# MachinePerceptionLab/Attentive_DFPrior

Hardware: AMD Instinct MI355X
Metric: rendered rays/sec (64 samples/ray), Replica room0 (higher is better)
Workload: dtype f32 via f16x3 split (3 f16 MFMA products per f32 product: 22-bit products, f32 accumulate); 1 GPU; room0 640x480 render_img, 64 spp (48+16), synthetic box room, seed-0 random decoders, grids at the REFERENCE init (N(0,.01), high N(0,1e-4)); stage color, ray_batch_size 100000 (per-batch far clamp, rendered as one call with a depth maximum per 100 000-ray segment), ONE frame per step; samples_per_ray=64

## Files before the change

### attentive_dfprior_amd/csrc/adfp_decode_g.h

```cpp
#pragma once
#include "adfp_decode_h.h"

__host__ __device__ constexpr int unit16(int k) { return 16 * ((k & 7) >> 2) + 4 * (k >> 3) + (k & 3); }

template <int CDIM, int NOUT>
struct DecLayoutG {
    using F = DecLayout<CDIM, NOUT>;
    static constexpr int KG_E = 3;
    static constexpr int KG_C = CDIM / 32;
    __host__ __device__ static constexpr int kg(int i) { return i == 0 ? KG_E : (i == 3 ? KG_E + 1 : 1); }
    static constexpr int P_BM = 0;
    __host__ __device__ static constexpr int layer_words(int i) { return kg(i) * 1024 + 32 + KG_C * 1024 + 32; }
    __host__ __device__ static constexpr int P_WP(int i) {
        int o = 384;
        for (int k = 0; k < i; ++k) o += layer_words(k);
        return o;
    }
    __host__ __device__ static constexpr int P_BP(int i) { return P_WP(i) + kg(i) * 1024; }
    __host__ __device__ static constexpr int P_WC(int i) { return P_BP(i) + 32; }
    __host__ __device__ static constexpr int P_BC(int i) { return P_WC(i) + KG_C * 1024; }
    static constexpr int P_WO = P_WP(5);
    static constexpr int P_BO = P_WO + NOUT * 32;
    static constexpr int P_FLAG = P_BO + 4;
    static constexpr int NFLAG = (((P_FLAG + 511) / 256) + 3) & ~3;
    static constexpr int P_TOTAL = P_FLAG + NFLAG;
    static_assert((P_TOTAL + 255) / 256 <= NFLAG, "one flag word per pack block");
};

template <int CDIM, int NOUT>
__device__ HSrc dec_g_src(int t) {
    using L = DecLayoutG<CDIM, NOUT>;
    using F = DecLayout<CDIM, NOUT>;
    if (t < 384) {
        const int row = t >> 2, c = t & 3;
        const int f = (row & ~31) + unit16(row & 31);
        return HSrc{0, (f < 93 && c < 3) ? F::F_EB + c * 93 + f : -1, -1};
    }
#pragma unroll
    for (int i = 0; i < 5; ++i) {
        if (t < L::P_BP(i) || (t >= L::P_WC(i) && t < L::P_BC(i))) {
            const bool fc = t >= L::P_WC(i);
            const int u = t - (fc ? L::P_WC(i) : L::P_WP(i));
            const int grp = u >> 10, ob = (u >> 9) & 1, part = (u >> 8) & 1, g = (u >> 6) & 3, row = 16 * ob + ((u >> 2) & 15), jp = (u & 3) * 2;
            int src[2];
#pragma unroll
            for (int e = 0; e < 2; ++e) {
                int col = 32 * grp + unit16(8 * g + jp + e);
                if (fc) src[e] = F::F_FC(i) + row * CDIM + col;
                else {
                    if (i == 0) { if (col >= 93) col = -1; }
                    else if (i == 3) { if (col < 96) { if (col >= 93) col = -1; } else col = 93 + (col - 96); }
                    src[e] = col < 0 ? -1 : F::F_PL(i) + row * F::in_dim(i) + col;
                }
            }
            return HSrc{1 + part, src[0], src[1]};
        }
        if (t < L::P_WC(i)) return HSrc{0, F::F_PL(i) + 32 * F::in_dim(i) + (t - L::P_BP(i)), -1};
        if (t < L::P_BC(i) + 32) return HSrc{0, F::F_FC(i) + 32 * CDIM + (t - L::P_BC(i)), -1};
    }
    if (t < L::P_BO) {
        const int u = t - L::P_WO;
        return HSrc{0, F::F_OW + u, -1};
    }
    const int o = t - L::P_BO;
    return HSrc{0, o < NOUT ? F::F_OB + o : -1, -1};
}

template <int CDIM, int NOUT>
ADFP_DEV void pack_decoder_g_block(int blk, const float* __restrict__ flat, unsigned* __restrict__ packed, int* __restrict__ status, int bit) {
    using L = DecLayoutG<CDIM, NOUT>;
    const int t = blk * 256 + (int)threadIdx.x;
    HSrc s{0, -1, -1};
    float a = 0.f, b = 0.f;
    if (t < L::P_FLAG) {
        s = dec_g_src<CDIM, NOUT>(t);
        a = s.s0 < 0 ? 0.f : flat[s.s0]; b = s.s1 < 0 ? 0.f : flat[s.s1];
    }
    pack_block_flag(!(fmaxf(fabsf(a), fabsf(b)) < 65504.0f), packed + L::P_FLAG + blk, status, bit);
    if (t >= L::P_FLAG) return;
    if (s.kind == 0) { packed[t] = s.s0 < 0 ? 0u : __float_as_uint(a); return; }
    a = f16_clamp(a); b = f16_clamp(b);
    const float ah = f16_hi_part(a), bh = f16_hi_part(b);
    _Float16 x, y;
    if (s.kind == 1) { x = (_Float16)ah; y = (_Float16)bh; }
    else { x = (_Float16)(a - ah); y = (_Float16)(b - bh); }
    packed[t] = (unsigned)__builtin_bit_cast(unsigned short, x) | ((unsigned)__builtin_bit_cast(unsigned short, y) << 16);
}
template <int CDIM, int NOUT>
__global__ void k_pack_decoder_g(const float* __restrict__ flat, unsigned* __restrict__ packed, int* __restrict__ status, int bit) { pack_decoder_g_block<CDIM, NOUT>((int)blockIdx.x, flat, packed, status, bit); }

typedef float f32x4g __attribute__((ext_vector_type(4)));

ADFP_DEV void swap_halves(float& x, float& y) {
    const auto r = __builtin_amdgcn_permlane32_swap(__float_as_uint(x), __float_as_uint(y), false, false);
    x = __uint_as_float(r[0]); y = __uint_as_float(r[1]);
}

template <int NG>
ADFP_DEV void mfma_chain_g(f32x4g acc[2][2], const unsigned* __restrict__ w, const f16x8 (*xh)[2], const f16x8 (*xl)[2]) {
#pragma unroll
    for (int kg = 0; kg < NG; ++kg) {
#pragma unroll
        for (int ob = 0; ob < 2; ++ob) {
            const f16x8 ah = __builtin_bit_cast(f16x8, *(const u32x4*)(w + kg * 1024 + ob * 512));
            const f16x8 al = __builtin_bit_cast(f16x8, *(const u32x4*)(w + kg * 1024 + ob * 512 + 256));
#pragma unroll
            for (int pb = 0; pb < 2; ++pb) {
                acc[ob][pb] = __builtin_amdgcn_mfma_f32_16x16x32_f16(ah, xh[kg][pb], acc[ob][pb], 0, 0, 0);
                acc[ob][pb] = __builtin_amdgcn_mfma_f32_16x16x32_f16(ah, xl[kg][pb], acc[ob][pb], 0, 0, 0);
                acc[ob][pb] = __builtin_amdgcn_mfma_f32_16x16x32_f16(al, xh[kg][pb], acc[ob][pb], 0, 0, 0);
            }
        }
    }
    __builtin_amdgcn_sched_barrier(0);
}

ADFP_DEV void row_store(float* p, const f32x4 v) {
    *(f32x4*)p = v;
}
template <int CDIM, int NOUT, int TRAIN = 0>
ADFP_DEV void decode_net_g(const unsigned* __restrict__ ldsu, const GridDev& grid, const GridDev& grid1, const float pn[3], const float (*pf)[3],
                           int lane, float& amax, float (*out)[NOUT], unsigned* __restrict__ mw, float* srow0, unsigned rowbits) {
    using L = DecLayoutG<CDIM, NOUT>;
    using ST = DecStage<CDIM>;
    const int g = lane >> 4;
    float* srow[2] = {nullptr, nullptr};
    if constexpr (TRAIN) {
        srow[0] = (rowbits & 1u) ? srow0 : nullptr;
        srow[1] = (rowbits & 2u) ? srow0 + 16 * ST::NXM : nullptr;
    }
    const unsigned* wl = ldsu + 4 * lane;
    const float* b4 = (const float*)ldsu + 4 * g;
    const float* brow = (const float*)ldsu + 32 * g;
    f16x8 ch[L::KG_C][2], cl[L::KG_C][2];
#pragma unroll
    for (int kc = 0; kc < L::KG_C; ++kc) {
        float c[16];
        gather16(kc == 0 ? grid : grid1, pn, g & 1, c);
        float x[8] = {c[0], c[1], c[2], c[3], c[8], c[9], c[10], c[11]};
        float y[8] = {c[4], c[5], c[6], c[7], c[12], c[13], c[14], c[15]};
#pragma unroll
        for (int s = 0; s < 8; ++s) swap_halves(x[s], y[s]);
        if constexpr (TRAIN) {
            static_assert(!TRAIN || CDIM == 32, "training rows: 32-channel decoders");
            if (srow[0]) { row_store(srow[0] + ST::xm(ST::SC) + 4 * g, f32x4{x[0], x[1], x[2], x[3]}); row_store(srow[0] + ST::xm(ST::SC) + 16 + 4 * g, f32x4{x[4], x[5], x[6], x[7]}); }
            if (srow[1]) { row_store(srow[1] + ST::xm(ST::SC) + 4 * g, f32x4{y[0], y[1], y[2], y[3]}); row_store(srow[1] + ST::xm(ST::SC) + 16 + 4 * g, f32x4{y[4], y[5], y[6], y[7]}); }
        }
        split8(x, ch[kc][0], cl[kc][0], amax);
        split8(y, ch[kc][1], cl[kc][1], amax);
    }
    f16x8 eh[L::KG_E][2], el[L::KG_E][2];
#pragma unroll
    for (int kg = 0; kg < L::KG_E; ++kg) {
        float e0[8], e1[8];
#pragma unroll
        for (int j = 0; j < 8; ++j) {
            const f32x4 bm = *(const f32x4*)(brow + L::P_BM + (32 * kg + j) * 4);
            e0[j] = adfp_sinf(fmaf(pf[0][2], bm.z, fmaf(pf[0][1], bm.y, pf[0][0] * bm.x)));
            e1[j] = adfp_sinf(fmaf(pf[1][2], bm.z, fmaf(pf[1][1], bm.y, pf[1][0] * bm.x)));
        }
        split8<false>(e0, eh[kg][0], el[kg][0], amax);
        split8<false>(e1, eh[kg][1], el[kg][1], amax);
    }
    __builtin_amdgcn_sched_barrier(0);
    f32x4g acc[2][2];
    f16x8 hh[1][2], hl[1][2];
    unsigned mk[3] = {0u, 0u, 0u};
#pragma unroll
    for (int i = 0; i < 5; ++i) {
#pragma unroll
        for (int ob = 0; ob < 2; ++ob) { const f32x4 t = *(const f32x4*)(b4 + L::P_BP(i) + 16 * ob); acc[ob][0] = t; acc[ob][1] = t; }
        if (i == 0) mfma_chain_g<L::KG_E>(acc, wl + L::P_WP(0), eh, el);
        else if (i == 3) {
            mfma_chain_g<L::KG_E>(acc, wl + L::P_WP(3), eh, el);
            mfma_chain_g<1>(acc, wl + L::P_WP(3) + L::KG_E * 1024, hh, hl);
        } else mfma_chain_g<1>(acc, wl + L::P_WP(i), hh, hl);
#pragma unroll
        for (int ob = 0; ob < 2; ++ob) {
            const f32x4 t = *(const f32x4*)(b4 + L::P_BC(i) + 16 * ob);
#pragma unroll
            for (int pb = 0; pb < 2; ++pb)
#pragma unroll
                for (int r = 0; r < 4; ++r) {
                    const float v = relu_f(acc[ob][pb][r]);
                    if constexpr (TRAIN) mk[i >> 1] = __builtin_amdgcn_alignbit(mk[i >> 1], 0u - __float_as_uint(v), 31);
                    acc[ob][pb][r] = v + t[r];
                }
        }
        mfma_chain_g<L::KG_C>(acc, wl + L::P_WC(i), ch, cl);
        if constexpr (TRAIN) {
#pragma unroll
            for (int pb = 0; pb < 2; ++pb) if (srow[pb]) {
                row_store(srow[pb] + ST::xm(ST::SH(i)) + 4 * g, f32x4{acc[0][pb][0], acc[0][pb][1], acc[0][pb][2], acc[0][pb][3]});
                row_store(srow[pb] + ST::xm(ST::SH(i)) + 16 + 4 * g, f32x4{acc[1][pb][0], acc[1][pb][1], acc[1][pb][2], acc[1][pb][3]});
            }
        }
        if (i < 4) {
#pragma unroll
            for (int pb = 0; pb < 2; ++pb) {
                const float t[8] = {acc[0][pb][0], acc[0][pb][1], acc[0][pb][2], acc[0][pb][3],
                                    acc[1][pb][0], acc[1][pb][1], acc[1][pb][2], acc[1][pb][3]};
                split8(t, hh[0][pb], hl[0][pb], amax);
            }
        }
    }
#pragma unroll
    for (int o = 0; o < NOUT; ++o) {
        const f32x4 w0 = *(const f32x4*)(b4 + L::P_WO + 32 * o), w1 = *(const f32x4*)(b4 + L::P_WO + 32 * o + 16);
#pragma unroll
        for (int pb = 0; pb < 2; ++pb) {
            float s = 0.f;
#pragma unroll
            for (int r = 0; r < 4; ++r) s = fmaf(acc[0][pb][r], w0[r], s);
#pragma unroll
            for (int r = 0; r < 4; ++r) s = fmaf(acc[1][pb][r], w1[r], s);
            s += __shfl_xor(s, 16);
            s += __shfl_xor(s, 32);
            out[pb][o] = s + ((const float*)ldsu)[L::P_BO + o];
        }
    }
    if constexpr (TRAIN) {
        const int sh = 4 * (g >> 1);
        unsigned wpb[2][3];
#pragma unroll
        for (int pb = 0; pb < 2; ++pb) {
            unsigned f[5];
#pragma unroll
            for (int i = 0; i < 5; ++i) {
                const unsigned m16 = (i == 4 || (i & 1)) ? (mk[i >> 1] & 0xFFFFu) : (mk[i >> 1] >> 16);
                const unsigned n0 = (m16 >> (12 - 4 * pb)) & 0xFu, n1 = (m16 >> (4 - 4 * pb)) & 0xFu;
                f[i] = (n0 << (12 - sh)) | (n1 << (4 - sh));
            }
            wpb[pb][0] = f[0] | (f[1] << 16); wpb[pb][1] = f[2] | (f[3] << 16); wpb[pb][2] = f[4];
        }
#pragma unroll
        for (int k = 0; k < 3; ++k) {
            const auto r = __builtin_amdgcn_permlane32_swap(wpb[0][k], wpb[1][k], false, false);
            mw[k] = r[0] | r[1];
        }
    }
}

template <int NT>
__global__ __launch_bounds__(NT, NT / 256) void k_decode_lc16(DecodeLCArgs a) {
    using LL = DecLayoutG<32, 1>;
    using LC = DecLayoutG<32, 4>;
    __shared__ __attribute__((aligned(16))) unsigned lds_all[LL::P_TOTAL + LC::P_TOTAL];
    __shared__ int s_next;
    __shared__ unsigned long long s_ring[ADFP_POOL_RING];
    unsigned* lds_low = lds_all;
    unsigned* lds_col = lds_all + LL::P_TOTAL;
    image_to_lds<NT, LL::P_TOTAL / 4>(lds_low, a.packed_low);
    image_to_lds<NT, LC::P_TOTAL / 4>(lds_col, a.packed_color);
    if (threadIdx.x == 0) s_next = NT / 64;
    if (threadIdx.x < ADFP_POOL_RING) s_ring[threadIdx.x] = 0ull;
    __syncthreads();
    const int lane = threadIdx.x & 63, n = lane & 15, g = lane >> 4;
    const int count = a.P.n;
    const int ntiles = (count + 31) >> 5;
    const TilePlan plan = tile_plan(ntiles, (int)gridDim.x, NT / 64, a.pool != nullptr);
    float amax_low = image_out_of_range<LL::P_FLAG, LL::NFLAG>(lds_low) ? INFINITY : 0.f;
    float amax_col = image_out_of_range<LC::P_FLAG, LC::NFLAG>(lds_col) ? INFINITY : 0.f;
    for (int j = threadIdx.x >> 6, tile; (tile = claim_tile_pool<NT / 64>(j, &s_next, s_ring, plan, ntiles, a.pool, a.status)) >= 0;) {
        const int idx = tile * 32 + 16 * (g >> 1) + n;
        const bool valid = idx < count;
        const int q = valid ? idx : 0;
        float pn[3], pf[2][3];
        bool pnan, keep_occ;
        {
            double pt[3];
            load_point(a.P, q, pt);
            normalize3(a.nb, pt, pn);
            const float f0 = (float)pt[0], f1 = (float)pt[1], f2 = (float)pt[2];
            pnan = (pt[0] != pt[0]) | (pt[1] != pt[1]) | (pt[2] != pt[2]);
            const unsigned f = a.flags ? a.flags[q] : 0u;
            keep_occ = (f & ADFP_F_BAND) || in_bound(pt, a.b) || !a.apply_bound;
            pf[0][0] = f0; pf[0][1] = f1; pf[0][2] = f2; pf[1][0] = f0; pf[1][1] = f1; pf[1][2] = f2;
        }
#pragma unroll
        for (int k = 0; k < 3; ++k) swap_halves(pf[0][k], pf[1][k]);
        float occ[2][1], rgb[2][4];
        int off_low = 0, off_col = LL::P_TOTAL;
        asm volatile("" : "+v"(off_low), "+v"(off_col));
        decode_net_g<32, 1>(lds_all + off_low, a.g_low, a.g_low, pn, pf, lane, amax_low, occ, nullptr, nullptr, 0u);
        asm volatile("" : "+v"(pn[0]), "+v"(pn[1]), "+v"(pn[2]), "+v"(occ[0][0]), "+v"(occ[1][0]));
        __builtin_amdgcn_sched_barrier(0);
        decode_net_g<32, 4>(lds_all + off_col, a.g_color, a.g_color, pn, pf, lane, amax_col, rgb, nullptr, nullptr, 0u);
        if (valid && (g & 1) == 0) {
            const int pb = g >> 1;
            const float nanv = __builtin_nanf("");
            const float o = pnan ? nanv : (keep_occ ? (pb ? occ[1][0] : occ[0][0]) : 100.f);
            const f32x4 c4 = pb ? f32x4{rgb[1][0], rgb[1][1], rgb[1][2], o} : f32x4{rgb[0][0], rgb[0][1], rgb[0][2], o};
            *(f32x4*)(a.raw + 4ll * q) = pnan ? f32x4{nanv, nanv, nanv, o} : c4;
            if (a.write_w) a.w[q] = 1.f;
        }
    }
    report_range(a.status, amax_low, ADFP_STATUS_F16_RANGE_LOW, a.call_flag);
    report_range(a.status, amax_col, ADFP_STATUS_F16_RANGE_COLOR, a.call_flag);
}

struct DecodeLCTrainArgs {
    DecodeLCArgs f;
    unsigned* masks_low; unsigned* masks_color;
    float* act_low; float* act_color;
    int split_networks;
};
template <int NT, bool SPLIT = false>
__global__ __launch_bounds__(NT, NT / 256) void k_decode_lc16_train(DecodeLCTrainArgs t) {
    const DecodeLCArgs& a = t.f;
    using LL = DecLayoutG<32, 1>;
    using LC = DecLayoutG<32, 4>;
    using ST = DecStage<32>;
    __shared__ __attribute__((aligned(16))) unsigned lds_all[LL::P_TOTAL + LC::P_TOTAL];
    __shared__ int s_next;
    unsigned* lds_low = lds_all;
    unsigned* lds_col = lds_all + LL::P_TOTAL;
    image_to_lds<NT, LL::P_TOTAL / 4>(lds_low, a.packed_low);
    image_to_lds<NT, LC::P_TOTAL / 4>(lds_col, a.packed_color);
    if (threadIdx.x == 0) s_next = NT / 64;
    __syncthreads();
    const int lane = threadIdx.x & 63, n = lane & 15, g = lane >> 4;
    const int count = a.P.n;
    const int ntiles = (count + 31) >> 5;
    float amax_low = image_out_of_range<LL::P_FLAG, LL::NFLAG>(lds_low) ? INFINITY : 0.f;
    float amax_col = image_out_of_range<LC::P_FLAG, LC::NFLAG>(lds_col) ? INFINITY : 0.f;
    constexpr bool split = SPLIT;
    const int njobs = split ? 2 * ntiles : ntiles;
    for (int j = threadIdx.x >> 6, job; (job = claim_tile<NT / 64>(j, &s_next, njobs)) >= 0;) {
        const int tile = split ? job >> 1 : job;
        const bool do_low = !split || (job & 1) == 0, do_col = !split || (job & 1) == 1;
        const int idx = tile * 32 + 16 * (g >> 1) + n;
        const bool valid = idx < count;
        const int q = valid ? idx : 0;
        float pn[3], pf[2][3];
        bool pnan, keep_occ;
        {
            double pt[3];
            load_point(a.P, q, pt);
            normalize3(a.nb, pt, pn);
            pnan = (pt[0] != pt[0]) | (pt[1] != pt[1]) | (pt[2] != pt[2]);
            const float f0 = pnan ? 0.f : (float)pt[0], f1 = pnan ? 0.f : (float)pt[1], f2 = pnan ? 0.f : (float)pt[2];
            const unsigned f = a.flags ? a.flags[q] : 0u;
            keep_occ = (f & ADFP_F_BAND) || in_bound(pt, a.b) || !a.apply_bound;
            pf[0][0] = f0; pf[0][1] = f1; pf[0][2] = f2; pf[1][0] = f0; pf[1][1] = f1; pf[1][2] = f2;
        }
#pragma unroll
        for (int k = 0; k < 3; ++k) swap_halves(pf[0][k], pf[1][k]);
        const int i0 = tile * 32 + n;
        const unsigned rowbits = (i0 < count ? 1u : 0u) | (i0 + 16 < count ? 2u : 0u);
        float occ[2][1], rgb[2][4];
        unsigned mw[3];
        int off_low = 0, off_col = LL::P_TOTAL;
        asm volatile("" : "+v"(off_low), "+v"(off_col));
        if constexpr (split) {
            occ[0][0] = 0.f; occ[1][0] = 0.f;
#pragma unroll
            for (int k = 0; k < 4; ++k) { rgb[0][k] = 0.f; rgb[1][k] = 0.f; }
        }
        if (do_low) {
            decode_net_g<32, 1, 1>(lds_all + off_low, a.g_low, a.g_low, pn, pf, lane, amax_low, occ, mw, t.act_low + (long long)i0 * ST::NXM, t.act_low ? rowbits : 0u);
            if (valid) { unsigned* mrow = t.masks_low + ((long long)q * 2 + (g & 1)) * 3; mrow[0] = mw[0]; mrow[1] = mw[1]; mrow[2] = mw[2]; }
        }
        asm volatile("" : "+v"(pn[0]), "+v"(pn[1]), "+v"(pn[2]), "+v"(occ[0][0]), "+v"(occ[1][0]));
        __builtin_amdgcn_sched_barrier(0);
        if (do_col) {
            decode_net_g<32, 4, 1>(lds_all + off_col, a.g_color, a.g_color, pn, pf, lane, amax_col, rgb, mw, t.act_color + (long long)i0 * ST::NXM, t.act_color ? rowbits : 0u);
            if (valid) { unsigned* mrow = t.masks_color + ((long long)q * 2 + (g & 1)) * 3; mrow[0] = mw[0]; mrow[1] = mw[1]; mrow[2] = mw[2]; }
        }
        if (valid && (g & 1) == 0) {
            const int pb = g >> 1;
            const float nanv = __builtin_nanf("");
            const float o = pnan ? nanv : (keep_occ ? (pb ? occ[1][0] : occ[0][0]) : 100.f);
            const f32x4 c4 = pb ? f32x4{rgb[1][0], rgb[1][1], rgb[1][2], o} : f32x4{rgb[0][0], rgb[0][1], rgb[0][2], o};
            const f32x4 row = pnan ? f32x4{nanv, nanv, nanv, o} : c4;
            if (!split) {
                *(f32x4*)(a.raw + 4ll * q) = row;
                if (a.write_w) a.w[q] = 1.f;
            } else if (do_low) {
                a.raw[4ll * q + 3] = row.w;
                if (a.write_w) a.w[q] = 1.f;
            } else {
                a.raw[4ll * q] = row.x; a.raw[4ll * q + 1] = row.y; a.raw[4ll * q + 2] = row.z;
            }
        }
    }
    report_range(a.status, amax_low, ADFP_STATUS_F16_RANGE_LOW, a.call_flag);
    report_range(a.status, amax_col, ADFP_STATUS_F16_RANGE_COLOR, a.call_flag);
}

template <int NT>
__global__ __launch_bounds__(NT, NT / 256) void k_decode_high_g(DecodeArgs a) {
    using L = DecLayoutG<64, 1>;
    __shared__ __attribute__((aligned(16))) unsigned ldsu[L::P_TOTAL];
    __shared__ int s_next;
    __shared__ unsigned long long s_ring[ADFP_POOL_RING];
    image_to_lds<NT, L::P_TOTAL / 4>(ldsu, a.packed);
    if (threadIdx.x == 0) s_next = NT / 64;
    if (threadIdx.x < ADFP_POOL_RING) s_ring[threadIdx.x] = 0ull;
    __syncthreads();
    const int lane = threadIdx.x & 63, n = lane & 15, g = lane >> 4;
    const int count = *a.count_ptr;
    const int ntiles = (count + 31) >> 5;
    const TilePlan plan = tile_plan(ntiles, (int)gridDim.x, NT / 64, a.pool != nullptr);
    float amax = image_out_of_range<L::P_FLAG, L::NFLAG>(ldsu) ? INFINITY : 0.f;
    for (int j = threadIdx.x >> 6, tile; (tile = claim_tile_pool<NT / 64>(j, &s_next, s_ring, plan, ntiles, a.pool, a.status)) >= 0;) {
        const int idx = tile * 32 + 16 * (g >> 1) + n;
        const bool valid = idx < count;
        const int q = a.list[valid ? idx : 0];
        float pn[3], pf[2][3];
        bool pnan;
        const float low_occ = (a.single || !valid) ? 0.f : a.raw[4ll * q + 3];
        {
            double pt[3];
            load_point(a.P, q, pt);
            normalize3(a.nb, pt, pn);
            const float f0 = (float)pt[0], f1 = (float)pt[1], f2 = (float)pt[2];
            pnan = (pt[0] != pt[0]) | (pt[1] != pt[1]) | (pt[2] != pt[2]);
            pf[0][0] = f0; pf[0][1] = f1; pf[0][2] = f2; pf[1][0] = f0; pf[1][1] = f1; pf[1][2] = f2;
        }
#pragma unroll
        for (int k = 0; k < 3; ++k) swap_halves(pf[0][k], pf[1][k]);
        float out[2][1];
        decode_net_g<64, 1>(ldsu, a.g0, a.g1, pn, pf, lane, amax, out, nullptr, nullptr, 0u);
        if (valid && (g & 1) == 0) {
            const float o = g >> 1 ? out[1][0] : out[0][0];
            const float v = pnan ? __builtin_nanf("") : o;
            a.att_occ[idx] = a.single ? v : v + low_occ;
        }
    }
    report_range(a.status, amax, ADFP_STATUS_F16_RANGE_HIGH, a.call_flag);
}

struct AttLayoutG {
    using F = AttLayout;
    static constexpr int P_A0 = 0;
    static constexpr int P_W1 = 256;
    static constexpr int P_B1 = P_W1 + 4 * 2 * 1024;
    static constexpr int P_W2 = P_B1 + 128;
    static constexpr int P_B2 = P_W2 + 4 * 4 * 1024;
    static constexpr int P_W3 = P_B2 + 128;
    static constexpr int P_B3 = P_W3 + 2 * 4 * 1024;
    static constexpr int P_WO = P_B3 + 64;
    static constexpr int P_BO = P_WO + 128;
    static constexpr int P_FLAG = P_BO + 4;
    static constexpr int NFLAG = (((P_FLAG + 511) / 256) + 3) & ~3;
    static constexpr int P_TOTAL = P_FLAG + NFLAG;
    static_assert((P_TOTAL + 255) / 256 <= NFLAG, "one flag word per pack block");
};

__device__ HSrc att_g_src(int t) {
    using L = AttLayoutG;
    using F = AttLayout;
    if (t < L::P_W1) {
        const int row = t >> 2, c = t & 3;
        const int u = (row & ~31) + unit16(row & 31);
        return HSrc{0, c < 2 ? F::F_W0 + u * 2 + c : (c == 2 ? F::F_B0 + u : -1), -1};
    }
    auto chain = [](int u, int ngrp, int base, int ld) {
        const int blk = u / (ngrp * 1024), v = u % (ngrp * 1024);
        const int grp = v >> 10, ob = (v >> 9) & 1, part = (v >> 8) & 1, g = (v >> 6) & 3, row = 32 * blk + 16 * ob + ((v >> 2) & 15), jp = (v & 3) * 2;
        return HSrc{1 + part, base + row * ld + 32 * grp + unit16(8 * g + jp), base + row * ld + 32 * grp + unit16(8 * g + jp + 1)};
    };
    if (t < L::P_B1) return chain(t - L::P_W1, 2, F::F_W1, 64);
    if (t < L::P_W2) return HSrc{0, F::F_B1 + (t - L::P_B1), -1};
    if (t < L::P_B2) return chain(t - L::P_W2, 4, F::F_W2, 128);
    if (t < L::P_W3) return HSrc{0, F::F_B2 + (t - L::P_B2), -1};
    if (t < L::P_B3) return chain(t - L::P_W3, 4, F::F_W3, 128);
    if (t < L::P_WO) return HSrc{0, F::F_B3 + (t - L::P_B3), -1};
    if (t < L::P_BO) return HSrc{0, F::F_WO + (t - L::P_WO), -1};
    const int o = t - L::P_BO;
    return HSrc{0, o < 2 ? F::F_BO + o : -1, -1};
}

ADFP_DEV void pack_attention_g_block(int blk, const float* __restrict__ flat, unsigned* __restrict__ packed, int* __restrict__ status) {
    using L = AttLayoutG;
    const int t = blk * 256 + (int)threadIdx.x;
    HSrc s{0, -1, -1};
    float a = 0.f, b = 0.f;
    if (t < L::P_FLAG) {
        s = att_g_src(t);
        a = s.s0 < 0 ? 0.f : flat[s.s0]; b = s.s1 < 0 ? 0.f : flat[s.s1];
    }
    pack_block_flag(!(fmaxf(fabsf(a), fabsf(b)) < 65504.0f), packed + L::P_FLAG + blk, status, ADFP_STATUS_F16_RANGE_ATT);
    if (t >= L::P_FLAG) return;
    if (s.kind == 0) { packed[t] = s.s0 < 0 ? 0u : __float_as_uint(a); return; }
    a = f16_clamp(a); b = f16_clamp(b);
    const float ah = f16_hi_part(a), bh = f16_hi_part(b);
    _Float16 x, y;
    if (s.kind == 1) { x = (_Float16)ah; y = (_Float16)bh; }
    else { x = (_Float16)(a - ah); y = (_Float16)(b - bh); }
    packed[t] = (unsigned)__builtin_bit_cast(unsigned short, x) | ((unsigned)__builtin_bit_cast(unsigned short, y) << 16);
}
__global__ void k_pack_attention_g(const float* __restrict__ flat, unsigned* __restrict__ packed, int* __restrict__ status) { pack_attention_g_block((int)blockIdx.x, flat, packed, status); }

template <int NT>
__global__ __launch_bounds__(NT) void k_attention_g(AttArgs a) {
    using A = AttLayoutG;
    __shared__ __attribute__((aligned(16))) unsigned ldsu[A::P_TOTAL];
    __shared__ int s_next;
    __shared__ unsigned long long s_ring[ADFP_POOL_RING];
    image_to_lds<NT, A::P_TOTAL / 4>(ldsu, a.packed);
    if (threadIdx.x == 0) s_next = NT / 64;
    if (threadIdx.x < ADFP_POOL_RING) s_ring[threadIdx.x] = 0ull;
    __syncthreads();
    const float* lds = (const float*)ldsu;
    const int lane = threadIdx.x & 63, n = lane & 15, g = lane >> 4;
    const unsigned* wl = ldsu + 4 * lane;
    const float* b4 = lds + 4 * g;
    const float* arow = lds + 32 * g;
    const int count = a.count_ptr ? *a.count_ptr : a.n_rows;
    const int ntiles = (count + 31) >> 5;
    const TilePlan plan = tile_plan(ntiles, (int)gridDim.x, NT / 64, a.pool != nullptr);
    float amax = image_out_of_range<A::P_FLAG, A::NFLAG>(ldsu) ? INFINITY : 0.f;
    for (int j = threadIdx.x >> 6, tile; (tile = claim_tile_pool<NT / 64>(j, &s_next, s_ring, plan, ntiles, a.pool, a.status)) >= 0;) {
        int idx[2]; bool valid[2]; float occ[2], u[2];
#pragma unroll
        for (int pb = 0; pb < 2; ++pb) {
            idx[pb] = tile * 32 + 16 * pb + n;
            valid[pb] = idx[pb] < count;
            const int ii = valid[pb] ? idx[pb] : 0;
            occ[pb] = a.att_occ[ii]; u[pb] = a.att_u[ii];
        }
        f16x8 xh[4][2], xl[4][2];
#pragma unroll
        for (int b = 0; b < 2; ++b) {
            float t0[8], t1[8];
#pragma unroll
            for (int k = 0; k < 8; ++k) {
                const f32x4 t = *(const f32x4*)(arow + A::P_A0 + (32 * b + k) * 4);
                t0[k] = relu_f(fmaf(u[0], t.y, fmaf(occ[0], t.x, t.z)));
                t1[k] = relu_f(fmaf(u[1], t.y, fmaf(occ[1], t.x, t.z)));
            }
            split8(t0, xh[b][0], xl[b][0], amax);
            split8(t1, xh[b][1], xl[b][1], amax);
        }
        __builtin_amdgcn_sched_barrier(0);
        f16x8 yh[4][2], yl[4][2];
#pragma unroll
        for (int blk = 0; blk < 4; ++blk) {
            f32x4g acc[2][2];
#pragma unroll
            for (int ob = 0; ob < 2; ++ob) { const f32x4 t = *(const f32x4*)(b4 + A::P_B1 + 32 * blk + 16 * ob); acc[ob][0] = t; acc[ob][1] = t; }
            mfma_chain_g<2>(acc, wl + A::P_W1 + blk * 2 * 1024, xh, xl);
#pragma unroll
            for (int pb = 0; pb < 2; ++pb) {
                const float t[8] = {relu_f(acc[0][pb][0]), relu_f(acc[0][pb][1]), relu_f(acc[0][pb][2]), relu_f(acc[0][pb][3]),
                                    relu_f(acc[1][pb][0]), relu_f(acc[1][pb][1]), relu_f(acc[1][pb][2]), relu_f(acc[1][pb][3])};
                split8(t, yh[blk][pb], yl[blk][pb], amax);
            }
        }
#pragma unroll
        for (int blk = 0; blk < 4; ++blk) {
            f32x4g acc[2][2];
#pragma unroll
            for (int ob = 0; ob < 2; ++ob) { const f32x4 t = *(const f32x4*)(b4 + A::P_B2 + 32 * blk + 16 * ob); acc[ob][0] = t; acc[ob][1] = t; }
            mfma_chain_g<4>(acc, wl + A::P_W2 + blk * 4 * 1024, yh, yl);
#pragma unroll
            for (int pb = 0; pb < 2; ++pb) {
                const float t[8] = {relu_f(acc[0][pb][0]), relu_f(acc[0][pb][1]), relu_f(acc[0][pb][2]), relu_f(acc[0][pb][3]),
                                    relu_f(acc[1][pb][0]), relu_f(acc[1][pb][1]), relu_f(acc[1][pb][2]), relu_f(acc[1][pb][3])};
                split8(t, xh[blk][pb], xl[blk][pb], amax);
            }
        }
        float l0[2] = {0.f, 0.f}, l1[2] = {0.f, 0.f};
#pragma unroll
        for (int blk = 0; blk < 2; ++blk) {
            f32x4g acc[2][2];
#pragma unroll
            for (int ob = 0; ob < 2; ++ob) { const f32x4 t = *(const f32x4*)(b4 + A::P_B3 + 32 * blk + 16 * ob); acc[ob][0] = t; acc[ob][1] = t; }
            mfma_chain_g<4>(acc, wl + A::P_W3 + blk * 4 * 1024, xh, xl);
#pragma unroll
            for (int ob = 0; ob < 2; ++ob) {
                const f32x4 w0 = *(const f32x4*)(b4 + A::P_WO + 32 * blk + 16 * ob), w1 = *(const f32x4*)(b4 + A::P_WO + 64 + 32 * blk + 16 * ob);
#pragma unroll
                for (int pb = 0; pb < 2; ++pb)
#pragma unroll
                    for (int r = 0; r < 4; ++r) {
                        const float v = relu_f(acc[ob][pb][r]);
                        l0[pb] = fmaf(v, w0[r], l0[pb]);
                        l1[pb] = fmaf(v, w1[r], l1[pb]);
                    }
            }
        }
#pragma unroll
        for (int pb = 0; pb < 2; ++pb) {
            l0[pb] += __shfl_xor(l0[pb], 16); l0[pb] += __shfl_xor(l0[pb], 32);
            l1[pb] += __shfl_xor(l1[pb], 16); l1[pb] += __shfl_xor(l1[pb], 32);
        }
        if (g < 2 && valid[g]) {
            const float a0l = l0[g] + lds[A::P_BO], a1l = l1[g] + lds[A::P_BO + 1];
            const float m = fmaxf(a0l, a1l);
            const float e0 = expf(a0l - m), e1 = expf(a1l - m);
            const float den = e0 + e1;
            const float a0 = e0 / den, a1 = e1 / den;
            const float fused = a0 * occ[g] + a1 * u[g];
            const int ii = idx[g];
            const int q = a.list ? a.list[ii] : ii;
            const bool inb = !a.flags || (a.flags[q] & ADFP_F_INBOUND) != 0;
            a.raw[4ll * q + 3] = (inb || !a.apply_bound) ? fused : 100.f;
            a.w[q] = a1;
        }
    }
    report_range(a.status, amax, ADFP_STATUS_F16_RANGE_ATT, a.call_flag);
}
```

Baseline: 58.25 million rays/s.

## Software-pipeline attention MLP epilogues under next block's MFMA chain

Restructures the attention MLP layers so each output block's ReLU and f16 hi/lo split (or output dot product) for the previous block is interleaved piecewise into the MFMA chain of the next block, using double-buffered accumulators. It adds explicit sched_group_barrier ordering to place VALU and LDS reads between MFMAs, and prefetches weight fragments one step ahead. The aim is to hide the epilogue VALU latency behind matrix work. In exchange it raises register pressure and ties performance to the compiler honouring the schedule hints; the split also now computes the low part with an fma against -1 rather than the previous helper.

```diff
diff --git a/attentive_dfprior_amd/csrc/adfp_decode_g.h b/attentive_dfprior_amd/csrc/adfp_decode_g.h
--- a/attentive_dfprior_amd/csrc/adfp_decode_g.h
+++ b/attentive_dfprior_amd/csrc/adfp_decode_g.h
@@ -493,6 +493,96 @@
 }
 __global__ void k_pack_attention_g(const float* __restrict__ flat, unsigned* __restrict__ packed, int* __restrict__ status) { pack_attention_g_block((int)blockIdx.x, flat, packed, status); }
 
+struct AttNoPiece { ADFP_DEV void operator()(int) const {} };
+template <int NG, class Piece>
+ADFP_DEV void att_chain(f32x4g acc[2][2], const unsigned* __restrict__ w, const f16x8 (*xh)[2], const f16x8 (*xl)[2], Piece&& piece) {
+    constexpr int NP = 2 * NG, STEP = 12 * NG / 8;
+    f16x8 ah[NP], al[NP];
+    ah[0] = __builtin_bit_cast(f16x8, *(const u32x4*)w);
+    al[0] = __builtin_bit_cast(f16x8, *(const u32x4*)(w + 256));
+#pragma unroll
+    for (int p = 0; p < NP; ++p) {
+        const int kg = p >> 1, ob = p & 1;
+        if (p + 1 < NP) {
+            ah[p + 1] = __builtin_bit_cast(f16x8, *(const u32x4*)(w + (p + 1) * 512));
+            al[p + 1] = __builtin_bit_cast(f16x8, *(const u32x4*)(w + (p + 1) * 512 + 256));
+        }
+#pragma unroll
+        for (int pb = 0; pb < 2; ++pb) {
+            acc[ob][pb] = __builtin_amdgcn_mfma_f32_16x16x32_f16(ah[p], xh[kg][pb], acc[ob][pb], 0, 0, 0);
+            acc[ob][pb] = __builtin_amdgcn_mfma_f32_16x16x32_f16(ah[p], xl[kg][pb], acc[ob][pb], 0, 0, 0);
+            acc[ob][pb] = __builtin_amdgcn_mfma_f32_16x16x32_f16(al[p], xh[kg][pb], acc[ob][pb], 0, 0, 0);
+            if ((6 * p + 3 * pb + 3) % STEP == 0) piece((6 * p + 3 * pb + 3) / STEP - 1);
+        }
+    }
+}
+ADFP_DEV void att_bias(f32x4g acc[2][2], const float* __restrict__ b) {
+#pragma unroll
+    for (int ob = 0; ob < 2; ++ob) { const f32x4 t = *(const f32x4*)(b + 16 * ob); acc[ob][0] = t; acc[ob][1] = t; }
+}
+struct AttSplitPieces {
+    typedef _Float16 h2 __attribute__((ext_vector_type(2)));
+    const f32x4g (*acc)[2];
+    f16x8 *h, *l;
+    float& amax;
+    u32x4 uh[2], ul[2];
+    ADFP_DEV AttSplitPieces(const f32x4g (*acc_)[2], f16x8* h_, f16x8* l_, float& amax_) : acc(acc_), h(h_), l(l_), amax(amax_) {}
+    ADFP_DEV void operator()(int k) {
+        const int pb = k >> 2, j = k & 3, ob = j >> 1, r = 2 * (j & 1);
+        unsigned m1 = 0xBC00BC00u;
+        asm("" : "+v"(m1));
+        const h2 neg1 = __builtin_bit_cast(h2, m1);
+        const float a = relu_f(acc[ob][pb][r]), b = relu_f(acc[ob][pb][r + 1]);
+        amax = __builtin_fmaxf(__builtin_fmaxf(__builtin_fabsf(a), __builtin_fabsf(b)), amax);
+        const h2 hp = __builtin_bit_cast(h2, __builtin_amdgcn_cvt_pkrtz(a, b));
+        h2 lp;
+        lp[0] = (_Float16)__builtin_fmaf((float)hp[0], (float)neg1[0], a);
+        lp[1] = (_Float16)__builtin_fmaf((float)hp[1], (float)neg1[0], b);
+        uh[pb][j] = __builtin_bit_cast(unsigned, hp);
+        ul[pb][j] = __builtin_bit_cast(unsigned, lp);
+        if (j == 3) {
+            h[pb] = __builtin_bit_cast(f16x8, uh[pb]);
+            l[pb] = __builtin_bit_cast(f16x8, ul[pb]);
+            asm("" : "+v"(amax));
+        }
+    }
+};
+struct AttOutPieces {
+    const f32x4g (*acc)[2];
+    const float* wo;
+    float *l0, *l1;
+    ADFP_DEV void operator()(int k) const {
+        const int ob = k >> 2, pb = (k >> 1) & 1, r0 = 2 * (k & 1);
+        const f32x4 w0 = *(const f32x4*)(wo + 16 * ob), w1 = *(const f32x4*)(wo + 64 + 16 * ob);
+#pragma unroll
+        for (int r = r0; r < r0 + 2; ++r) {
+            const float v = relu_f(acc[ob][pb][r]);
+            l0[pb] = fmaf(v, w0[r], l0[pb]);
+            l1[pb] = fmaf(v, w1[r], l1[pb]);
+        }
+    }
+};
+template <class Piece>
+ADFP_DEV void att_pieces(Piece&& piece) {
+#pragma unroll
+    for (int k = 0; k < 8; ++k) piece(k);
+}
+constexpr int ATT_FILL1 = 2, ATT_FILL2 = 1;
+template <int NG, int F, int XDS = 0>
+ADFP_DEV void att_stage_order(void) {
+    __builtin_amdgcn_sched_group_barrier(0x100, 4 + XDS, 0);
+#pragma unroll
+    for (int p = 0; p < 2 * NG; ++p) {
+#pragma unroll
+        for (int m = 0; m < 6; ++m) {
+            __builtin_amdgcn_sched_group_barrier(0x008, 1, 0);
+            if (m == 0 && p + 1 < 2 * NG) __builtin_amdgcn_sched_group_barrier(0x100, 2, 0);
+            __builtin_amdgcn_sched_group_barrier(0x002, F, 0);
+        }
+    }
+    __builtin_amdgcn_sched_barrier(0);
+}
+
 template <int NT>
 __global__ __launch_bounds__(NT) void k_attention_g(AttArgs a) {
     using A = AttLayoutG;
@@ -535,53 +625,38 @@
             split8(t1, xh[b][1], xl[b][1], amax);
         }
         __builtin_amdgcn_sched_barrier(0);
+        f32x4g acc[2][2][2];
         f16x8 yh[4][2], yl[4][2];
-#pragma unroll
-        for (int blk = 0; blk < 4; ++blk) {
-            f32x4g acc[2][2];
-#pragma unroll
-            for (int ob = 0; ob < 2; ++ob) { const f32x4 t = *(const f32x4*)(b4 + A::P_B1 + 32 * blk + 16 * ob); acc[ob][0] = t; acc[ob][1] = t; }
-            mfma_chain_g<2>(acc, wl + A::P_W1 + blk * 2 * 1024, xh, xl);
-#pragma unroll
-            for (int pb = 0; pb < 2; ++pb) {
-                const float t[8] = {relu_f(acc[0][pb][0]), relu_f(acc[0][pb][1]), relu_f(acc[0][pb][2]), relu_f(acc[0][pb][3]),
-                                    relu_f(acc[1][pb][0]), relu_f(acc[1][pb][1]), relu_f(acc[1][pb][2]), relu_f(acc[1][pb][3])};
-                split8(t, yh[blk][pb], yl[blk][pb], amax);
-            }
-        }
-#pragma unroll
-        for (int blk = 0; blk < 4; ++blk) {
-            f32x4g acc[2][2];
-#pragma unroll
-            for (int ob = 0; ob < 2; ++ob) { const f32x4 t = *(const f32x4*)(b4 + A::P_B2 + 32 * blk + 16 * ob); acc[ob][0] = t; acc[ob][1] = t; }
-            mfma_chain_g<4>(acc, wl + A::P_W2 + blk * 4 * 1024, yh, yl);
-#pragma unroll
-            for (int pb = 0; pb < 2; ++pb) {
-                const float t[8] = {relu_f(acc[0][pb][0]), relu_f(acc[0][pb][1]), relu_f(acc[0][pb][2]), relu_f(acc[0][pb][3]),
-                                    relu_f(acc[1][pb][0]), relu_f(acc[1][pb][1]), relu_f(acc[1][pb][2]), relu_f(acc[1][pb][3])};
-                split8(t, xh[blk][pb], xl[blk][pb], amax);
-            }
-        }
+        att_bias(acc[0], b4 + A::P_B1);
+        att_chain<2>(acc[0], wl + A::P_W1, xh, xl, AttNoPiece());
+        __builtin_amdgcn_sched_barrier(0);
+#pragma unroll
+        for (int blk = 1; blk < 4; ++blk) {
+            att_bias(acc[blk & 1], b4 + A::P_B1 + 32 * blk);
+            att_chain<2>(acc[blk & 1], wl + A::P_W1 + blk * 2 * 1024, xh, xl, AttSplitPieces(acc[(blk - 1) & 1], yh[blk - 1], yl[blk - 1], amax));
+            att_stage_order<2, ATT_FILL1>();
+        }
+        att_pieces(AttSplitPieces(acc[1], yh[3], yl[3], amax));
+        __builtin_amdgcn_sched_barrier(0);
+        att_bias(acc[0], b4 + A::P_B2);
+        att_chain<4>(acc[0], wl + A::P_W2, yh, yl, AttNoPiece());
+        __builtin_amdgcn_sched_barrier(0);
+#pragma unroll
+        for (int blk = 1; blk < 4; ++blk) {
+            att_bias(acc[blk & 1], b4 + A::P_B2 + 32 * blk);
+            att_chain<4>(acc[blk & 1], wl + A::P_W2 + blk * 4 * 1024, yh, yl, AttSplitPieces(acc[(blk - 1) & 1], xh[blk - 1], xl[blk - 1], amax));
+            att_stage_order<4, ATT_FILL2>();
+        }
+        att_pieces(AttSplitPieces(acc[1], xh[3], xl[3], amax));
+        __builtin_amdgcn_sched_barrier(0);
         float l0[2] = {0.f, 0.f}, l1[2] = {0.f, 0.f};
-#pragma unroll
-        for (int blk = 0; blk < 2; ++blk) {
-            f32x4g acc[2][2];
-#pragma unroll
-            for (int ob = 0; ob < 2; ++ob) { const f32x4 t = *(const f32x4*)(b4 + A::P_B3 + 32 * blk + 16 * ob); acc[ob][0] = t; acc[ob][1] = t; }
-            mfma_chain_g<4>(acc, wl + A::P_W3 + blk * 4 * 1024, xh, xl);
-#pragma unroll
-            for (int ob = 0; ob < 2; ++ob) {
-                const f32x4 w0 = *(const f32x4*)(b4 + A::P_WO + 32 * blk + 16 * ob), w1 = *(const f32x4*)(b4 + A::P_WO + 64 + 32 * blk + 16 * ob);
-#pragma unroll
-                for (int pb = 0; pb < 2; ++pb)
-#pragma unroll
-                    for (int r = 0; r < 4; ++r) {
-                        const float v = relu_f(acc[ob][pb][r]);
-                        l0[pb] = fmaf(v, w0[r], l0[pb]);
-                        l1[pb] = fmaf(v, w1[r], l1[pb]);
-                    }
-            }
-        }
+        att_bias(acc[0], b4 + A::P_B3);
+        att_chain<4>(acc[0], wl + A::P_W3, xh, xl, AttNoPiece());
+        __builtin_amdgcn_sched_barrier(0);
+        att_bias(acc[1], b4 + A::P_B3 + 32);
+        att_chain<4>(acc[1], wl + A::P_W3 + 4 * 1024, xh, xl, AttOutPieces{acc[0], b4 + A::P_WO, l0, l1});
+        att_stage_order<4, ATT_FILL2, 4>();
+        att_pieces(AttOutPieces{acc[1], b4 + A::P_WO + 32, l0, l1});
 #pragma unroll
         for (int pb = 0; pb < 2; ++pb) {
             l0[pb] += __shfl_xor(l0[pb], 16); l0[pb] += __shfl_xor(l0[pb], 32);
```

Result: no change. 58.83 million rays/s, median of 6 (+1.0%).
